# brdav/refign

Measured on AMD Instinct MI355X. Metric: image-pairs/s (align+seg fwd+bwd, 1080x1920), higher is better.
Workload: dtype bf16

## Files before the change

### refign_amd/csrc/kvpath.hip

```cpp
#include "common.h"
#include "elem.h"
#include "mfma.h"

namespace rfn {

constexpr int kKvBlocks = 3;
constexpr int kKvSmall = 128;
constexpr int kKvPack = 4096;
constexpr int kKvSPitch = 64 + 8;

template <int C, int R, int NB> struct KvGeom {
  static constexpr int ROWS = 32 * NB;
  static constexpr int KSTEP = C <= 128 ? 128 : 64;
  static constexpr int XP = KSTEP + 8, YP = C + 8;
  static constexpr int YBYTES = ROWS * YP * 2;
  static constexpr int XBYTES = R > 1 ? ROWS * XP * 2 : 0;
  static constexpr int WSCR = 32 * ((R > 1 && KSTEP > 64 ? KSTEP : 64) + 8) * 2;
  static constexpr int SBYTES = 4 * WSCR;
  static constexpr int LDS = YBYTES + 2 * XBYTES + SBYTES;
  static_assert(C % 64 == 0 && (R == 1 || (R * C) % KSTEP == 0), "a K-step never straddles a run of the gather");
  static_assert(LDS <= 160 * 1024, "LDS");
};

template <int DT, int C, int R, int NB>
__global__ __launch_bounds__(256) void kvpath_kernel(const uint16_t* __restrict__ X, const uint16_t* __restrict__ Wsr,
                                                     const uint16_t* __restrict__ bsr, const float* __restrict__ gamma,
                                                     const float* __restrict__ beta, float eps, const uint16_t* __restrict__ Wkv,
                                                     const uint16_t* __restrict__ bkv, unsigned char* __restrict__ kr,
                                                     unsigned char* __restrict__ vt, uint16_t* __restrict__ kvout, int B, int H,
                                                     int W, int Wr, int Nkv, int nkblk) {
  using E = Elem<DT>;
  using vec8 = typename E::vec8;
  using G = KvGeom<C, R, NB>;
  constexpr int kKvBlocks = NB, kKvRows = G::ROWS;
  constexpr int CB = C / 32, HEADS = C / 64, NCH = 2 * HEADS;
  constexpr int YP = G::YP;
  __shared__ __attribute__((aligned(16))) unsigned char smem[G::LDS];
  uint16_t* yt = (uint16_t*)smem;
  unsigned char* scr = smem + G::YBYTES + 2 * G::XBYTES;

  const int t = threadIdx.x, lane = t & 63, col = lane & 31, g = lane >> 5;
  const int wave = __builtin_amdgcn_readfirstlane(t >> 6);
  const int nblocks = B * nkblk, gb0 = blockIdx.x * kKvBlocks;
  auto row_of = [&](int tr, int& b, int& blk, int& row) {
    const int gb = gb0 + (tr >> 5);
    b = gb / nkblk;
    blk = gb - b * nkblk;
    row = blk * 32 + (tr & 31);
    return gb < nblocks && row < Nkv;
  };

  if constexpr (R > 1) {
    constexpr int KSTEP = G::KSTEP, XP = G::XP, NKS = KSTEP / 16, K1 = R * R * C;
    constexpr int PPR = KSTEP / 8, RPP = 256 / PPR, NI = kKvRows / RPP;
    constexpr int NCW = CB >= 4 ? (CB + 3) / 4 : 1, NTW = CB >= 4 ? kKvBlocks : (kKvBlocks + 1) / 2;
    static_assert(CB >= 4 || CB == 2, "wave map");
    const int sub = t % PPR, rb = t / PPR;
    unsigned xo[NI];
#pragma unroll
    for (int i = 0; i < NI; ++i) {
      int b, blk, row;
      const bool ok = row_of(rb + RPP * i, b, blk, row);
      const int oy = row / Wr, ox = row - oy * Wr;
      xo[i] = (ok ? (unsigned)(((b * H + oy * R) * W + ox * R) * C) : 0u) + sub * 8;
    }
    auto fetch_x = [&](int k0, u32x4(&rx)[NI]) {
      const int ry = k0 / (R * C);
      const unsigned off = (unsigned)(ry * W * C + (k0 - ry * R * C));
#pragma unroll
      for (int i = 0; i < NI; ++i) rx[i] = *(const u32x4*)(X + (xo[i] + off));
    };
    auto stash_x = [&](int buf, const u32x4(&rx)[NI]) {
      unsigned char* xs = smem + G::YBYTES + buf * G::XBYTES + (rb * XP + sub * 8) * 2;
#pragma unroll
      for (int i = 0; i < NI; ++i) *(u32x4*)(xs + RPP * i * XP * 2) = rx[i];
    };
    int cbc[NCW], tbc[NTW];
    bool cb_ok[NCW], tb_ok[NTW];
#pragma unroll
    for (int i = 0; i < NCW; ++i) {
      const int cb = CB >= 4 ? wave + 4 * i : (wave & 1);
      cb_ok[i] = cb < CB;
      cbc[i] = min(cb, CB - 1);
    }
#pragma unroll
    for (int j = 0; j < NTW; ++j) {
      const int tb = CB >= 4 ? j : (wave >> 1) + 2 * j;
      tb_ok[j] = tb < kKvBlocks;
      tbc[j] = min(tb, kKvBlocks - 1);
    }
    constexpr int WP = KSTEP + 8, PPW = KSTEP / 8, RPI = 64 / PPW;
    static_assert(32 / RPI == NKS, "instructions per block");
    const int wr = lane / PPW, wp = lane % PPW;
    const uint16_t* wrow[NCW];
#pragma unroll
    for (int i = 0; i < NCW; ++i) wrow[i] = Wsr + (long)(cbc[i] * 32 + wr) * K1 + wp * 8;
    auto fetch_w = [&](int k0, vec8(&wf)[NCW][NKS]) {
#pragma unroll
      for (int i = 0; i < NCW; ++i)
#pragma unroll
        for (int q = 0; q < NKS; ++q) wf[i][q] = *(const vec8*)(wrow[i] + (long)q * RPI * K1 + k0);
    };
    unsigned char* wscr = scr + wave * G::WSCR;
    auto to_frags = [&](const vec8(&raw)[NKS], vec8(&fr)[NKS]) {
      asm volatile("" ::: "memory");
#pragma unroll
      for (int q = 0; q < NKS; ++q) *(vec8*)(wscr + ((q * RPI + wr) * WP + wp * 8) * 2) = raw[q];
      asm volatile("" ::: "memory");
#pragma unroll
      for (int ks = 0; ks < NKS; ++ks) fr[ks] = *(const vec8*)(wscr + (col * WP + ks * 16 + 8 * g) * 2);
      asm volatile("" ::: "memory");
    };
    f32x16 acc[NCW][NTW];
#pragma unroll
    for (int i = 0; i < NCW; ++i)
#pragma unroll
      for (int j = 0; j < NTW; ++j)
#pragma unroll
        for (int r = 0; r < 16; ++r) acc[i][j][r] = 0.f;
    constexpr int nk = K1 / KSTEP;
    auto kstep = [&](int s, vec8(&cur)[NCW][NKS], vec8(&far)[NCW][NKS], const u32x4(&rnext)[NI], u32x4(&rfar)[NI]) {
      const bool more = s + 1 < nk;
      if (s + 2 < nk) {
        fetch_x((s + 2) * KSTEP, rfar);
        fetch_w((s + 2) * KSTEP, far);
      }
      const unsigned char* xs = smem + G::YBYTES + (s & 1) * G::XBYTES;
      auto xfrag = [&](int j, int ks) { return *(const vec8*)(xs + ((tbc[j] * 32 + col) * XP + ks * 16 + 8 * g) * 2); };
      vec8 xall[NCW > 1 ? NKS : 1][NTW];
      if constexpr (NCW > 1) {
#pragma unroll
        for (int ks = 0; ks < NKS; ++ks)
#pragma unroll
          for (int j = 0; j < NTW; ++j) xall[ks][j] = xfrag(j, ks);
      }
#pragma unroll
      for (int i = 0; i < NCW; ++i) {
        vec8 wfr[NKS];
        to_frags(cur[i], wfr);
#pragma unroll
        for (int ks = 0; ks < NKS; ++ks)
#pragma unroll
          for (int j = 0; j < NTW; ++j) acc[i][j] = E::mma(wfr[ks], NCW > 1 ? xall[NCW > 1 ? ks : 0][j] : xfrag(j, ks), acc[i][j]);
      }
      if (more) stash_x((s + 1) & 1, rnext);
      __syncthreads();
    };
    vec8 wf0[NCW][NKS], wf1[NCW][NKS], wf2[NCW][NKS];
    u32x4 rxa[NI], rxb[NI];
    static_assert(nk >= 2, "two steps in flight");
    fetch_x(0, rxa);
    fetch_w(0, wf0);
    fetch_x(KSTEP, rxb);
    fetch_w(KSTEP, wf1);
    stash_x(0, rxa);
    __syncthreads();
#pragma unroll 1
    for (int s = 0; s < nk; s += 6) {
      kstep(s, wf0, wf2, rxb, rxa);
      if (s + 1 < nk) kstep(s + 1, wf1, wf0, rxa, rxb);
      if (s + 2 < nk) kstep(s + 2, wf2, wf1, rxb, rxa);
      if (s + 3 < nk) kstep(s + 3, wf0, wf2, rxa, rxb);
      if (s + 4 < nk) kstep(s + 4, wf1, wf0, rxb, rxa);
      if (s + 5 < nk) kstep(s + 5, wf2, wf1, rxa, rxb);
    }
#pragma unroll
    for (int i = 0; i < NCW; ++i)
#pragma unroll
      for (int j = 0; j < NTW; ++j) {
        if (!(cb_ok[i] && tb_ok[j])) continue;
        const int tok = tbc[j] * 32 + col;
#pragma unroll
        for (int q = 0; q < 4; ++q) {
          const int n0 = cbc[i] * 32 + 8 * q + 4 * g;
          float bf[4];
          unpack4<DT>(*(const u32x2*)(bsr + n0), bf);
          *(u32x2*)(yt + tok * YP + n0) = pack4<DT>(acc[i][j][4 * q] + bf[0], acc[i][j][4 * q + 1] + bf[1],
                                                   acc[i][j][4 * q + 2] + bf[2], acc[i][j][4 * q + 3] + bf[3]);
        }
      }
    __syncthreads();
    {
      constexpr int LPR = C <= 64 ? 8 : (C <= 128 ? 16 : (C <= 256 ? 32 : 64)), RPW = 64 / LPR;
      const int ls = lane % LPR, grp = lane / LPR, c = ls * 8;
      const bool act = c < C;
      float gm[8], bt[8];
#pragma unroll
      for (int h = 0; h < 2; ++h) {
        const f32x4 a = *(const f32x4*)(gamma + (act ? c : 0) + 4 * h), b = *(const f32x4*)(beta + (act ? c : 0) + 4 * h);
#pragma unroll
        for (int e = 0; e < 4; ++e) {
          gm[4 * h + e] = a[e];
          bt[4 * h + e] = b[e];
        }
      }
      const float invC = 1.0f / (float)C;
#pragma unroll 1
      for (int it = 0; it < kKvRows / (4 * RPW); ++it) {
        uint16_t* p = yt + ((it * 4 + wave) * RPW + grp) * YP + (act ? c : 0);
        float v[8];
        if (act) load8<DT>(p, v);
        else {
#pragma unroll
          for (int i = 0; i < 8; ++i) v[i] = 0.0f;
        }
        float s = 0.0f;
#pragma unroll
        for (int i = 0; i < 8; ++i) s += v[i];
#pragma unroll
        for (int o = LPR / 2; o > 0; o >>= 1) s += __shfl_xor(s, o, 64);
        const float mu = s * invC;
        float q = 0.0f;
#pragma unroll
        for (int i = 0; i < 8; ++i) {
          const float d = act ? v[i] - mu : 0.0f;
          q = fmaf(d, d, q);
        }
#pragma unroll
        for (int o = LPR / 2; o > 0; o >>= 1) q += __shfl_xor(q, o, 64);
        const float rs = rsqrtf(q * invC + eps);
        if (act) {
          float o[8];
#pragma unroll
          for (int i = 0; i < 8; ++i) o[i] = fmaf((v[i] - mu) * rs, gm[i], bt[i]);
          const u32x2 lo = pack4<DT>(o[0], o[1], o[2], o[3]), hi = pack4<DT>(o[4], o[5], o[6], o[7]);
          *(u32x4*)p = u32x4{lo[0], lo[1], hi[0], hi[1]};
        }
      }
    }
    __syncthreads();
  } else {
    constexpr int PPR = C / 8;
    for (int p = t; p < kKvRows * PPR; p += 256) {
      const int tr = p / PPR, sub = p - tr * PPR;
      int b, blk, row;
      u32x4 v = {0u, 0u, 0u, 0u};
      if (row_of(tr, b, blk, row)) v = *(const u32x4*)(X + ((long)b * Nkv + row) * C + sub * 8);
      *(u32x4*)(yt + tr * YP + sub * 8) = v;
    }
    __syncthreads();
  }

  constexpr int NPASS = (NCH + 3) / 4;
#pragma unroll 1
  for (int pass = 0; pass < NPASS; ++pass) {
    const int hc = pass * 4 + wave;
    const bool hc_ok = hc < NCH;
    const int hcc = min(hc, NCH - 1);
    unsigned char* ws = scr + wave * G::WSCR;
    const int wr = lane >> 3, wp = lane & 7;
    const uint16_t* w2row = Wkv + (long)(hcc * 64 + wr) * C + wp * 8;
    auto fetch_w2 = [&](int k0, vec8(&wf)[2][4]) {
#pragma unroll
      for (int a = 0; a < 2; ++a)
#pragma unroll
        for (int q = 0; q < 4; ++q) wf[a][q] = *(const vec8*)(w2row + (long)(a * 32 + q * 8) * C + k0);
    };
    auto to_frags2 = [&](const vec8(&raw)[4], vec8(&fr)[4]) {
      asm volatile("" ::: "memory");
#pragma unroll
      for (int q = 0; q < 4; ++q) *(vec8*)(ws + ((q * 8 + wr) * kKvSPitch + wp * 8) * 2) = raw[q];
      asm volatile("" ::: "memory");
#pragma unroll
      for (int ks = 0; ks < 4; ++ks) fr[ks] = *(const vec8*)(ws + (col * kKvSPitch + ks * 16 + 8 * g) * 2);
      asm volatile("" ::: "memory");
    };
    f32x16 acc2[2][kKvBlocks];
#pragma unroll
    for (int a = 0; a < 2; ++a)
#pragma unroll
      for (int j = 0; j < kKvBlocks; ++j)
#pragma unroll
        for (int r = 0; r < 16; ++r) acc2[a][j][r] = 0.f;
    auto kstep2 = [&](int s, vec8(&cur)[2][4], vec8(&far)[2][4]) {
      if (s + 2 < HEADS) fetch_w2((s + 2) * 64, far);
      vec8 yf[4][kKvBlocks];
#pragma unroll
      for (int ks = 0; ks < 4; ++ks)
#pragma unroll
        for (int j = 0; j < kKvBlocks; ++j) yf[ks][j] = *(const vec8*)(yt + (j * 32 + col) * YP + s * 64 + ks * 16 + 8 * g);
#pragma unroll
      for (int a = 0; a < 2; ++a) {
        vec8 wfr[4];
        to_frags2(cur[a], wfr);
#pragma unroll
        for (int ks = 0; ks < 4; ++ks)
#pragma unroll
          for (int j = 0; j < kKvBlocks; ++j) acc2[a][j] = E::mma(wfr[ks], yf[ks][j], acc2[a][j]);
      }
    };
    vec8 v0[2][4], v1[2][4], v2[2][4];
    fetch_w2(0, v0);
    if (HEADS > 1) fetch_w2(64, v1);
#pragma unroll 1
    for (int s = 0; s < HEADS; s += 3) {
      kstep2(s, v0, v2);
      if (s + 1 < HEADS) kstep2(s + 1, v1, v0);
      if (s + 2 < HEADS) kstep2(s + 2, v2, v1);
    }
    const bool is_k = hc < HEADS;
#pragma unroll
    for (int j = 0; j < kKvBlocks; ++j) {
      int b, blk, row;
      const bool valid = row_of(j * 32 + col, b, blk, row);
      const bool live = hc_ok && gb0 + j < nblocks;
      const long pblk = ((long)(b * NCH + hcc) * nkblk + blk) * kKvPack;
#pragma unroll
      for (int a = 0; a < 2; ++a)
#pragma unroll
        for (int pr = 0; pr < 2; ++pr) {
          float ba[4], bb[4];
          const uint16_t* bp = bkv + hcc * 64 + a * 32 + 16 * pr + 4 * g;
          unpack4<DT>(*(const u32x2*)bp, ba);
          unpack4<DT>(*(const u32x2*)(bp + 8), bb);
          const u32x2 pa = pack4<DT>(acc2[a][j][8 * pr] + ba[0], acc2[a][j][8 * pr + 1] + ba[1], acc2[a][j][8 * pr + 2] + ba[2],
                                     acc2[a][j][8 * pr + 3] + ba[3]);
          const u32x2 pb = pack4<DT>(acc2[a][j][8 * pr + 4] + bb[0], acc2[a][j][8 * pr + 5] + bb[1], acc2[a][j][8 * pr + 6] + bb[2],
                                     acc2[a][j][8 * pr + 7] + bb[3]);
          auto r0 = __builtin_amdgcn_permlane32_swap(pa[0], pb[0], false, false);
          auto r1 = __builtin_amdgcn_permlane32_swap(pa[1], pb[1], false, false);
          const u32x4 o = valid ? u32x4{r0[0], r1[0], r0[1], r1[1]} : u32x4{0u, 0u, 0u, 0u};
          const int dc = a * 4 + 2 * pr + g;
          if (live && is_k) *(u32x4*)(kr + pblk + (dc * 32 + col) * 16) = o;
          if (live && valid && kvout != nullptr) *(u32x4*)(kvout + ((long)b * Nkv + row) * (2 * C) + hcc * 64 + dc * 8) = o;
          *(u32x4*)(ws + (col * kKvSPitch + dc * 8) * 2) = o;
        }
      __syncthreads();
      if (live && !is_k) {
        const uint16_t* sc = (const uint16_t*)ws + lane;
#pragma unroll
        for (int rq = 0; rq < 8; ++rq) {
          const unsigned h0 = sc[(4 * rq) * kKvSPitch], h1 = sc[(4 * rq + 1) * kKvSPitch], h2 = sc[(4 * rq + 2) * kKvSPitch],
                         h3 = sc[(4 * rq + 3) * kKvSPitch];
          *(u32x2*)(vt + pblk + (rq * 64 + lane) * 8) = u32x2{h0 | (h1 << 16), h2 | (h3 << 16)};
        }
      }
      __syncthreads();
    }
  }
}

template <int DT, int C, int R, int NB>
static int kvpath_launch(const void* x, const void* w_sr, const void* b_sr, const float* gamma, const float* beta, float eps,
                         const void* w_kv, const void* b_kv, void* k_rpack, void* v_tpack, void* kv_out, int B, int H, int W, int Nkv,
                         int nkblk, hipStream_t st) {
  const int tiles = cdiv((long)B * nkblk, NB);
  hipLaunchKernelGGL((kvpath_kernel<DT, C, R, NB>), dim3(tiles), dim3(256), 0, st, (const uint16_t*)x, (const uint16_t*)w_sr,
                     (const uint16_t*)b_sr, gamma, beta, eps, (const uint16_t*)w_kv, (const uint16_t*)b_kv, (unsigned char*)k_rpack,
                     (unsigned char*)v_tpack, (uint16_t*)kv_out, B, H, W, R > 1 ? W / R : 1, Nkv, nkblk);
  return check_launch("kvpath_kernel");
}

}

extern "C" int rfn_kv_path(const void* x, const void* w_sr, const void* b_sr, const float* gamma, const float* beta, float eps,
                           const void* w_kv, const void* b_kv, void* k_rpack, void* v_tpack, void* kv_out, int B, int H, int W, int C,
                           int r, int nkblk, int blocks_per_wg, int dtype, rfn_stream_t stream) {
  using namespace rfn;
  RFN_REQUIRE(x && w_kv && b_kv && k_rpack && v_tpack, "rfn_kv_path: null pointer");
  RFN_REQUIRE(r == 1 || (w_sr && b_sr && gamma && beta), "rfn_kv_path: r = %d needs the spatial-reduction and LayerNorm parameters", r);
  RFN_REQUIRE(B > 0 && H >= r && W >= r && r >= 1, "rfn_kv_path: B=%d H=%d W=%d r=%d", B, H, W, r);
  RFN_REQUIRE((long)B * H * W * C < (1L << 31), "rfn_kv_path: B*H*W*C = %ld (32-bit element offsets)", (long)B * H * W * C);
  const int Nkv = (H / r) * (W / r);
  RFN_REQUIRE(nkblk % 2 == 0 && (long)nkblk * 32 >= Nkv && (long)B * nkblk < (1L << 24),
              "rfn_kv_path: nkblk=%d (even, >= ceil(%d / 32))", nkblk, Nkv);
  hipStream_t st = (hipStream_t)stream;
  RFN_REQUIRE(blocks_per_wg == 0 || blocks_per_wg == 1 || blocks_per_wg == kKvBlocks, "rfn_kv_path: blocks_per_wg=%d (0, 1 or %d)",
              blocks_per_wg, kKvBlocks);
  const bool small = blocks_per_wg ? blocks_per_wg == 1 : cdiv((long)B * nkblk, kKvBlocks) < kKvSmall;
  return dt16(dtype, "rfn_kv_path", [&](auto dtc) {
    constexpr int DT = decltype(dtc)::value;
#define RFN_KV(CC, RR)                                                                                                   \
  if (C == CC && r == RR)                                                                                                \
    return small ? kvpath_launch<DT, CC, RR, 1>(x, w_sr, b_sr, gamma, beta, eps, w_kv, b_kv, k_rpack, v_tpack, kv_out, B, H, W, Nkv, \
                                                nkblk, st)                                                               \
                 : kvpath_launch<DT, CC, RR, kKvBlocks>(x, w_sr, b_sr, gamma, beta, eps, w_kv, b_kv, k_rpack, v_tpack, kv_out, B, H, \
                                                        W, Nkv, nkblk, st)
    RFN_KV(64, 8);
    RFN_KV(128, 4);
    RFN_KV(320, 2);
    RFN_KV(512, 1);
#undef RFN_KV
    return fail(RFN_EINVAL, "rfn_kv_path: (C, r) = (%d, %d): built for (64, 8), (128, 4), (320, 2), (512, 1)", C, r);
  });
}
```

Measured before the change: 17.73.

## Use eight waves per workgroup in the KV path for wide channel stages

For C >= 320 the KV-path kernel now launches 8 waves instead of 4. The spatial-reduction GEMM, LayerNorm and KV projection work is spread across the extra waves, and the weight prefetch is shortened to one step ahead to save registers. LayerNorm is unrolled over four rows so more work is in flight, per-wave pack barriers become compiler fences, and bias loads are hoisted. An optional s_memtime trace hook is added but compiled out by default. The extra waves trade register and LDS pressure and a shallower prefetch for more parallelism inside each block.

```diff
diff --git a/refign_amd/csrc/kvpath.hip b/refign_amd/csrc/kvpath.hip
--- a/refign_amd/csrc/kvpath.hip
+++ b/refign_amd/csrc/kvpath.hip
@@ -8,31 +8,38 @@
 constexpr int kKvSmall = 128;
 constexpr int kKvPack = 4096;
 constexpr int kKvSPitch = 64 + 8;
+constexpr int kKvStamps = 64;
 
 template <int C, int R, int NB> struct KvGeom {
+#ifdef RFN_KV_FOUR_WAVES
+  static constexpr int NW = 4;
+#else
+  static constexpr int NW = C >= 320 ? 8 : 4;
+#endif
   static constexpr int ROWS = 32 * NB;
   static constexpr int KSTEP = C <= 128 ? 128 : 64;
   static constexpr int XP = KSTEP + 8, YP = C + 8;
   static constexpr int YBYTES = ROWS * YP * 2;
   static constexpr int XBYTES = R > 1 ? ROWS * XP * 2 : 0;
   static constexpr int WSCR = 32 * ((R > 1 && KSTEP > 64 ? KSTEP : 64) + 8) * 2;
-  static constexpr int SBYTES = 4 * WSCR;
+  static constexpr int SBYTES = NW * WSCR;
   static constexpr int LDS = YBYTES + 2 * XBYTES + SBYTES;
   static_assert(C % 64 == 0 && (R == 1 || (R * C) % KSTEP == 0), "a K-step never straddles a run of the gather");
   static_assert(LDS <= 160 * 1024, "LDS");
 };
 
-template <int DT, int C, int R, int NB>
-__global__ __launch_bounds__(256) void kvpath_kernel(const uint16_t* __restrict__ X, const uint16_t* __restrict__ Wsr,
-                                                     const uint16_t* __restrict__ bsr, const float* __restrict__ gamma,
+template <int DT, int C, int R, int NB, bool TRACE = false>
+__global__ __launch_bounds__((64 * KvGeom<C, R, NB>::NW)) void kvpath_kernel(const uint16_t* __restrict__ X,
+                                                     const uint16_t* __restrict__ Wsr, const uint16_t* __restrict__ bsr, const float* __restrict__ gamma,
                                                      const float* __restrict__ beta, float eps, const uint16_t* __restrict__ Wkv,
                                                      const uint16_t* __restrict__ bkv, unsigned char* __restrict__ kr,
                                                      unsigned char* __restrict__ vt, uint16_t* __restrict__ kvout, int B, int H,
-                                                     int W, int Wr, int Nkv, int nkblk) {
+                                                     int W, int Wr, int Nkv, int nkblk, unsigned long long* __restrict__ trace) {
   using E = Elem<DT>;
   using vec8 = typename E::vec8;
   using G = KvGeom<C, R, NB>;
-  constexpr int kKvBlocks = NB, kKvRows = G::ROWS;
+  constexpr int kKvBlocks = NB, kKvRows = G::ROWS, NW = G::NW, NT = 64 * NW;
+  constexpr int AH = NW > 4 ? 1 : 2;
   constexpr int CB = C / 32, HEADS = C / 64, NCH = 2 * HEADS;
   constexpr int YP = G::YP;
   __shared__ __attribute__((aligned(16))) unsigned char smem[G::LDS];
@@ -50,17 +57,35 @@
     return gb < nblocks && row < Nkv;
   };
 
+  int tcount = 0;
+  auto stamp = [&]() {
+    if constexpr (TRACE) {
+      if (blockIdx.x == 0 && tcount < kKvStamps) {
+        unsigned long long tm;
+        __builtin_amdgcn_sched_barrier(0);
+        asm volatile("s_memtime %0\n\ts_waitcnt lgkmcnt(0)" : "=s"(tm)::"memory");
+        __builtin_amdgcn_sched_barrier(0);
+        if (lane == 0) trace[wave * kKvStamps + tcount] = tm;
+        ++tcount;
+      }
+    }
+  };
+  stamp();
+
   if constexpr (R > 1) {
     constexpr int KSTEP = G::KSTEP, XP = G::XP, NKS = KSTEP / 16, K1 = R * R * C;
-    constexpr int PPR = KSTEP / 8, RPP = 256 / PPR, NI = kKvRows / RPP;
-    constexpr int NCW = CB >= 4 ? (CB + 3) / 4 : 1, NTW = CB >= 4 ? kKvBlocks : (kKvBlocks + 1) / 2;
-    static_assert(CB >= 4 || CB == 2, "wave map");
+    constexpr int PPR = KSTEP / 8, RPP = NT / PPR, NI = (kKvRows + RPP - 1) / RPP;
+    constexpr bool XFULL = kKvRows % RPP == 0;
+    constexpr int NCW = CB >= 4 ? (CB + NW - 1) / NW : 1, NTW = CB >= 4 ? kKvBlocks : (kKvBlocks + 1) / 2;
+    static_assert((CB >= NW || CB == 2) && (NW == 4 || CB >= 4), "wave map");
     const int sub = t % PPR, rb = t / PPR;
     unsigned xo[NI];
+    bool xin[NI];
 #pragma unroll
     for (int i = 0; i < NI; ++i) {
       int b, blk, row;
-      const bool ok = row_of(rb + RPP * i, b, blk, row);
+      xin[i] = XFULL || rb + RPP * i < kKvRows;
+      const bool ok = row_of(rb + RPP * i, b, blk, row) && xin[i];
       const int oy = row / Wr, ox = row - oy * Wr;
       xo[i] = (ok ? (unsigned)(((b * H + oy * R) * W + ox * R) * C) : 0u) + sub * 8;
     }
@@ -73,13 +98,14 @@
     auto stash_x = [&](int buf, const u32x4(&rx)[NI]) {
       unsigned char* xs = smem + G::YBYTES + buf * G::XBYTES + (rb * XP + sub * 8) * 2;
 #pragma unroll
-      for (int i = 0; i < NI; ++i) *(u32x4*)(xs + RPP * i * XP * 2) = rx[i];
+      for (int i = 0; i < NI; ++i)
+        if (xin[i]) *(u32x4*)(xs + RPP * i * XP * 2) = rx[i];
     };
     int cbc[NCW], tbc[NTW];
     bool cb_ok[NCW], tb_ok[NTW];
 #pragma unroll
     for (int i = 0; i < NCW; ++i) {
-      const int cb = CB >= 4 ? wave + 4 * i : (wave & 1);
+      const int cb = CB >= 4 ? wave + NW * i : (wave & 1);
       cb_ok[i] = cb < CB;
       cbc[i] = min(cb, CB - 1);
     }
@@ -95,9 +121,9 @@
     const uint16_t* wrow[NCW];
 #pragma unroll
     for (int i = 0; i < NCW; ++i) wrow[i] = Wsr + (long)(cbc[i] * 32 + wr) * K1 + wp * 8;
-    auto fetch_w = [&](int k0, vec8(&wf)[NCW][NKS]) {
-#pragma unroll
-      for (int i = 0; i < NCW; ++i)
+    auto fetch_w = [&](auto nc, int k0, vec8(&wf)[NCW][NKS]) {
+#pragma unroll
+      for (int i = 0; i < decltype(nc)::value; ++i)
 #pragma unroll
         for (int q = 0; q < NKS; ++q) wf[i][q] = *(const vec8*)(wrow[i] + (long)q * RPI * K1 + k0);
     };
@@ -119,51 +145,72 @@
 #pragma unroll
         for (int r = 0; r < 16; ++r) acc[i][j][r] = 0.f;
     constexpr int nk = K1 / KSTEP;
-    auto kstep = [&](int s, vec8(&cur)[NCW][NKS], vec8(&far)[NCW][NKS], const u32x4(&rnext)[NI], u32x4(&rfar)[NI]) {
-      const bool more = s + 1 < nk;
-      if (s + 2 < nk) {
-        fetch_x((s + 2) * KSTEP, rfar);
-        fetch_w((s + 2) * KSTEP, far);
-      }
+    auto kstep = [&](auto nc, auto mode, int s, vec8(&cur)[NCW][NKS], vec8(&far)[NCW][NKS], const u32x4(&rnext)[NI],
+                     u32x4(&rfar)[NI]) {
+      constexpr int NC = decltype(nc)::value, MODE = decltype(mode)::value;
+      const bool more = MODE == 0 ? s + 1 < nk : MODE != 3;
+      if (MODE == 0 ? s + 2 < nk : MODE == 1) fetch_x((s + 2) * KSTEP, rfar);
+      if (MODE == 0 ? s + AH < nk : MODE != 3) fetch_w(nc, (s + AH) * KSTEP, far);
       const unsigned char* xs = smem + G::YBYTES + (s & 1) * G::XBYTES;
       auto xfrag = [&](int j, int ks) { return *(const vec8*)(xs + ((tbc[j] * 32 + col) * XP + ks * 16 + 8 * g) * 2); };
-      vec8 xall[NCW > 1 ? NKS : 1][NTW];
-      if constexpr (NCW > 1) {
+      constexpr bool XALL = NCW > 1 && NW == 4;
+      vec8 xall[XALL ? NKS : 1][NTW];
+      if constexpr (XALL) {
 #pragma unroll
         for (int ks = 0; ks < NKS; ++ks)
 #pragma unroll
           for (int j = 0; j < NTW; ++j) xall[ks][j] = xfrag(j, ks);
       }
 #pragma unroll
-      for (int i = 0; i < NCW; ++i) {
+      for (int i = 0; i < NC; ++i) {
         vec8 wfr[NKS];
         to_frags(cur[i], wfr);
 #pragma unroll
         for (int ks = 0; ks < NKS; ++ks)
 #pragma unroll
-          for (int j = 0; j < NTW; ++j) acc[i][j] = E::mma(wfr[ks], NCW > 1 ? xall[NCW > 1 ? ks : 0][j] : xfrag(j, ks), acc[i][j]);
+          for (int j = 0; j < NTW; ++j) acc[i][j] = E::mma(wfr[ks], XALL ? xall[XALL ? ks : 0][j] : xfrag(j, ks), acc[i][j]);
       }
       if (more) stash_x((s + 1) & 1, rnext);
       __syncthreads();
+      stamp();
     };
     vec8 wf0[NCW][NKS], wf1[NCW][NKS], wf2[NCW][NKS];
     u32x4 rxa[NI], rxb[NI];
     static_assert(nk >= 2, "two steps in flight");
-    fetch_x(0, rxa);
-    fetch_w(0, wf0);
-    fetch_x(KSTEP, rxb);
-    fetch_w(KSTEP, wf1);
-    stash_x(0, rxa);
-    __syncthreads();
+    auto product = [&](auto nc) {
+      fetch_x(0, rxa);
+      fetch_w(nc, 0, wf0);
+      fetch_x(KSTEP, rxb);
+      if constexpr (AH == 2) fetch_w(nc, KSTEP, wf1);
+      stash_x(0, rxa);
+      __syncthreads();
+      stamp();
+      using std::integral_constant;
+      if constexpr (AH == 1) {
+        static_assert(AH == 2 || nk % 2 == 0, "pairs of steps");
+        int s = 0;
 #pragma unroll 1
-    for (int s = 0; s < nk; s += 6) {
-      kstep(s, wf0, wf2, rxb, rxa);
-      if (s + 1 < nk) kstep(s + 1, wf1, wf0, rxa, rxb);
-      if (s + 2 < nk) kstep(s + 2, wf2, wf1, rxb, rxa);
-      if (s + 3 < nk) kstep(s + 3, wf0, wf2, rxa, rxb);
-      if (s + 4 < nk) kstep(s + 4, wf1, wf0, rxb, rxa);
-      if (s + 5 < nk) kstep(s + 5, wf2, wf1, rxa, rxb);
-    }
+        for (; s + 2 < nk; s += 2) {
+          kstep(nc, integral_constant<int, 1>{}, s, wf0, wf1, rxb, rxa);
+          kstep(nc, integral_constant<int, 1>{}, s + 1, wf1, wf0, rxa, rxb);
+        }
+        kstep(nc, integral_constant<int, 2>{}, s, wf0, wf1, rxb, rxa);
+        kstep(nc, integral_constant<int, 3>{}, s + 1, wf1, wf0, rxa, rxb);
+      } else {
+        constexpr integral_constant<int, 0> rt{};
+#pragma unroll 1
+        for (int s = 0; s < nk; s += 6) {
+          kstep(nc, rt, s, wf0, wf2, rxb, rxa);
+          if (s + 1 < nk) kstep(nc, rt, s + 1, wf1, wf0, rxa, rxb);
+          if (s + 2 < nk) kstep(nc, rt, s + 2, wf2, wf1, rxb, rxa);
+          if (s + 3 < nk) kstep(nc, rt, s + 3, wf0, wf2, rxa, rxb);
+          if (s + 4 < nk) kstep(nc, rt, s + 4, wf1, wf0, rxb, rxa);
+          if (s + 5 < nk) kstep(nc, rt, s + 5, wf2, wf1, rxa, rxb);
+        }
+      }
+    };
+    if (NW > 4 && NCW > 1 && !cb_ok[NCW - 1]) product(std::integral_constant<int, (NCW > 1 ? NCW - 1 : 1)>{});
+    else product(std::integral_constant<int, NCW>{});
 #pragma unroll
     for (int i = 0; i < NCW; ++i)
 #pragma unroll
@@ -180,6 +227,7 @@
         }
       }
     __syncthreads();
+    stamp();
     {
       constexpr int LPR = C <= 64 ? 8 : (C <= 128 ? 16 : (C <= 256 ? 32 : 64)), RPW = 64 / LPR;
       const int ls = lane % LPR, grp = lane / LPR, c = ls * 8;
@@ -195,43 +243,64 @@
         }
       }
       const float invC = 1.0f / (float)C;
+      constexpr int LNU = NW > 4 ? 4 : 1, ITER = kKvRows / (NW * RPW);
+      static_assert(ITER % LNU == 0, "rows in flight");
 #pragma unroll 1
-      for (int it = 0; it < kKvRows / (4 * RPW); ++it) {
-        uint16_t* p = yt + ((it * 4 + wave) * RPW + grp) * YP + (act ? c : 0);
-        float v[8];
-        if (act) load8<DT>(p, v);
-        else {
-#pragma unroll
-          for (int i = 0; i < 8; ++i) v[i] = 0.0f;
-        }
-        float s = 0.0f;
-#pragma unroll
-        for (int i = 0; i < 8; ++i) s += v[i];
-#pragma unroll
-        for (int o = LPR / 2; o > 0; o >>= 1) s += __shfl_xor(s, o, 64);
-        const float mu = s * invC;
-        float q = 0.0f;
-#pragma unroll
-        for (int i = 0; i < 8; ++i) {
-          const float d = act ? v[i] - mu : 0.0f;
-          q = fmaf(d, d, q);
-        }
-#pragma unroll
-        for (int o = LPR / 2; o > 0; o >>= 1) q += __shfl_xor(q, o, 64);
-        const float rs = rsqrtf(q * invC + eps);
+      for (int it = 0; it < ITER; it += LNU) {
+        uint16_t* p[LNU];
+        float v[LNU][8], s[LNU], q[LNU];
+#pragma unroll
+        for (int u = 0; u < LNU; ++u) {
+          p[u] = yt + (((it + u) * NW + wave) * RPW + grp) * YP + (act ? c : 0);
+          load8<DT>(p[u], v[u]);
+          s[u] = 0.0f;
+#pragma unroll
+          for (int i = 0; i < 8; ++i) {
+            v[u][i] = act ? v[u][i] : 0.0f;
+            s[u] += v[u][i];
+          }
+        }
+#pragma unroll
+        for (int o = LPR / 2; o > 0; o >>= 1)
+#pragma unroll
+          for (int u = 0; u < LNU; ++u) s[u] += __shfl_xor(s[u], o, 64);
+        float mu[LNU];
+#pragma unroll
+        for (int u = 0; u < LNU; ++u) {
+          mu[u] = s[u] * invC;
+          asm volatile("" : "+v"(mu[u]));
+          q[u] = 0.0f;
+#pragma unroll
+          for (int i = 0; i < 8; ++i) {
+            v[u][i] = act ? v[u][i] - mu[u] : 0.0f;
+            q[u] = fmaf(v[u][i], v[u][i], q[u]);
+          }
+        }
+#pragma unroll
+        for (int o = LPR / 2; o > 0; o >>= 1)
+#pragma unroll
+          for (int u = 0; u < LNU; ++u) q[u] += __shfl_xor(q[u], o, 64);
         if (act) {
-          float o[8];
-#pragma unroll
-          for (int i = 0; i < 8; ++i) o[i] = fmaf((v[i] - mu) * rs, gm[i], bt[i]);
-          const u32x2 lo = pack4<DT>(o[0], o[1], o[2], o[3]), hi = pack4<DT>(o[4], o[5], o[6], o[7]);
-          *(u32x4*)p = u32x4{lo[0], lo[1], hi[0], hi[1]};
+#pragma unroll
+          for (int u = 0; u < LNU; ++u) {
+            const float rs = rsqrtf(fmaf(q[u], invC, eps));
+            float o[8];
+#pragma unroll
+            for (int i = 0; i < 8; ++i) {
+              o[i] = fmaf(v[u][i] * rs, gm[i], bt[i]);
+              asm volatile("" : "+v"(o[i]));
+            }
+            const u32x2 lo = pack4<DT>(o[0], o[1], o[2], o[3]), hi = pack4<DT>(o[4], o[5], o[6], o[7]);
+            *(u32x4*)p[u] = u32x4{lo[0], lo[1], hi[0], hi[1]};
+          }
         }
       }
     }
     __syncthreads();
+    stamp();
   } else {
     constexpr int PPR = C / 8;
-    for (int p = t; p < kKvRows * PPR; p += 256) {
+    for (int p = t; p < kKvRows * PPR; p += NT) {
       const int tr = p / PPR, sub = p - tr * PPR;
       int b, blk, row;
       u32x4 v = {0u, 0u, 0u, 0u};
@@ -239,13 +308,19 @@
       *(u32x4*)(yt + tr * YP + sub * 8) = v;
     }
     __syncthreads();
+    stamp();
   }
 
-  constexpr int NPASS = (NCH + 3) / 4;
+  constexpr int NPASS = (NCH + NW - 1) / NW;
+  auto pack_sync = [&]() {
+    if constexpr (NW == 4) __syncthreads();
+    else asm volatile("" ::: "memory");
+  };
 #pragma unroll 1
   for (int pass = 0; pass < NPASS; ++pass) {
-    const int hc = pass * 4 + wave;
+    const int hc = pass * NW + wave;
     const bool hc_ok = hc < NCH;
+    if (NW > 4 && !hc_ok) break;
     const int hcc = min(hc, NCH - 1);
     unsigned char* ws = scr + wave * G::WSCR;
     const int wr = lane >> 3, wp = lane & 7;
@@ -272,13 +347,18 @@
       for (int j = 0; j < kKvBlocks; ++j)
 #pragma unroll
         for (int r = 0; r < 16; ++r) acc2[a][j][r] = 0.f;
-    auto kstep2 = [&](int s, vec8(&cur)[2][4], vec8(&far)[2][4]) {
-      if (s + 2 < HEADS) fetch_w2((s + 2) * 64, far);
-      vec8 yf[4][kKvBlocks];
-#pragma unroll
-      for (int ks = 0; ks < 4; ++ks)
-#pragma unroll
-        for (int j = 0; j < kKvBlocks; ++j) yf[ks][j] = *(const vec8*)(yt + (j * 32 + col) * YP + s * 64 + ks * 16 + 8 * g);
+    auto kstep2 = [&](auto mode, int s, vec8(&cur)[2][4], vec8(&far)[2][4]) {
+      constexpr int MODE = decltype(mode)::value;
+      if (MODE == 0 ? s + AH < HEADS : MODE == 1) fetch_w2((s + AH) * 64, far);
+      auto yfrag = [&](int j, int ks) { return *(const vec8*)(yt + (j * 32 + col) * YP + s * 64 + ks * 16 + 8 * g); };
+      constexpr bool YALL = NW == 4;
+      vec8 yf[YALL ? 4 : 1][kKvBlocks];
+      if constexpr (YALL) {
+#pragma unroll
+        for (int ks = 0; ks < 4; ++ks)
+#pragma unroll
+          for (int j = 0; j < kKvBlocks; ++j) yf[ks][j] = yfrag(j, ks);
+      }
 #pragma unroll
       for (int a = 0; a < 2; ++a) {
         vec8 wfr[4];
@@ -286,19 +366,49 @@
 #pragma unroll
         for (int ks = 0; ks < 4; ++ks)
 #pragma unroll
-          for (int j = 0; j < kKvBlocks; ++j) acc2[a][j] = E::mma(wfr[ks], yf[ks][j], acc2[a][j]);
+          for (int j = 0; j < kKvBlocks; ++j) acc2[a][j] = E::mma(wfr[ks], YALL ? yf[YALL ? ks : 0][j] : yfrag(j, ks), acc2[a][j]);
       }
     };
     vec8 v0[2][4], v1[2][4], v2[2][4];
     fetch_w2(0, v0);
-    if (HEADS > 1) fetch_w2(64, v1);
+    if (AH == 2 && HEADS > 1) fetch_w2(64, v1);
+    if constexpr (AH == 1) {
+      constexpr std::integral_constant<int, 1> req{};
+      constexpr std::integral_constant<int, 3> last{};
+      int s = 0;
 #pragma unroll 1
-    for (int s = 0; s < HEADS; s += 3) {
-      kstep2(s, v0, v2);
-      if (s + 1 < HEADS) kstep2(s + 1, v1, v0);
-      if (s + 2 < HEADS) kstep2(s + 2, v2, v1);
-    }
+      for (; s + 2 < HEADS; s += 2) {
+        kstep2(req, s, v0, v1);
+        kstep2(req, s + 1, v1, v0);
+      }
+      if constexpr (HEADS % 2 == 0) {
+        kstep2(req, s, v0, v1);
+        kstep2(last, s + 1, v1, v0);
+      } else {
+        kstep2(last, s, v0, v1);
+      }
+    } else {
+      constexpr std::integral_constant<int, 0> rt{};
+#pragma unroll 1
+      for (int s = 0; s < HEADS; s += 3) {
+        kstep2(rt, s, v0, v2);
+        if (s + 1 < HEADS) kstep2(rt, s + 1, v1, v0);
+        if (s + 2 < HEADS) kstep2(rt, s + 2, v2, v1);
+      }
+    }
+    stamp();
     const bool is_k = hc < HEADS;
+    u32x2 bpre[NW > 4 ? 2 : 1][2][2];
+    if constexpr (NW > 4) {
+#pragma unroll
+      for (int a = 0; a < 2; ++a)
+#pragma unroll
+        for (int pr = 0; pr < 2; ++pr) {
+          const uint16_t* bp = bkv + hcc * 64 + a * 32 + 16 * pr + 4 * g;
+          bpre[a][pr][0] = *(const u32x2*)bp;
+          bpre[a][pr][1] = *(const u32x2*)(bp + 8);
+        }
+    }
 #pragma unroll
     for (int j = 0; j < kKvBlocks; ++j) {
       int b, blk, row;
@@ -311,8 +421,8 @@
         for (int pr = 0; pr < 2; ++pr) {
           float ba[4], bb[4];
           const uint16_t* bp = bkv + hcc * 64 + a * 32 + 16 * pr + 4 * g;
-          unpack4<DT>(*(const u32x2*)bp, ba);
-          unpack4<DT>(*(const u32x2*)(bp + 8), bb);
+          unpack4<DT>(NW > 4 ? bpre[NW > 4 ? a : 0][pr][0] : *(const u32x2*)bp, ba);
+          unpack4<DT>(NW > 4 ? bpre[NW > 4 ? a : 0][pr][1] : *(const u32x2*)(bp + 8), bb);
           const u32x2 pa = pack4<DT>(acc2[a][j][8 * pr] + ba[0], acc2[a][j][8 * pr + 1] + ba[1], acc2[a][j][8 * pr + 2] + ba[2],
                                      acc2[a][j][8 * pr + 3] + ba[3]);
           const u32x2 pb = pack4<DT>(acc2[a][j][8 * pr + 4] + bb[0], acc2[a][j][8 * pr + 5] + bb[1], acc2[a][j][8 * pr + 6] + bb[2],
@@ -325,7 +435,7 @@
           if (live && valid && kvout != nullptr) *(u32x4*)(kvout + ((long)b * Nkv + row) * (2 * C) + hcc * 64 + dc * 8) = o;
           *(u32x4*)(ws + (col * kKvSPitch + dc * 8) * 2) = o;
         }
-      __syncthreads();
+      pack_sync();
       if (live && !is_k) {
         const uint16_t* sc = (const uint16_t*)ws + lane;
 #pragma unroll
@@ -335,24 +445,28 @@
           *(u32x2*)(vt + pblk + (rq * 64 + lane) * 8) = u32x2{h0 | (h1 << 16), h2 | (h3 << 16)};
         }
       }
-      __syncthreads();
-    }
+      pack_sync();
+    }
+    stamp();
   }
 }
 
+#ifndef RFN_KVPATH_KERNEL_ONLY
 template <int DT, int C, int R, int NB>
 static int kvpath_launch(const void* x, const void* w_sr, const void* b_sr, const float* gamma, const float* beta, float eps,
                          const void* w_kv, const void* b_kv, void* k_rpack, void* v_tpack, void* kv_out, int B, int H, int W, int Nkv,
                          int nkblk, hipStream_t st) {
   const int tiles = cdiv((long)B * nkblk, NB);
-  hipLaunchKernelGGL((kvpath_kernel<DT, C, R, NB>), dim3(tiles), dim3(256), 0, st, (const uint16_t*)x, (const uint16_t*)w_sr,
+  hipLaunchKernelGGL((kvpath_kernel<DT, C, R, NB>), dim3(tiles), dim3(64 * KvGeom<C, R, NB>::NW), 0, st, (const uint16_t*)x, (const uint16_t*)w_sr,
                      (const uint16_t*)b_sr, gamma, beta, eps, (const uint16_t*)w_kv, (const uint16_t*)b_kv, (unsigned char*)k_rpack,
-                     (unsigned char*)v_tpack, (uint16_t*)kv_out, B, H, W, R > 1 ? W / R : 1, Nkv, nkblk);
+                     (unsigned char*)v_tpack, (uint16_t*)kv_out, B, H, W, R > 1 ? W / R : 1, Nkv, nkblk, nullptr);
   return check_launch("kvpath_kernel");
 }
+#endif
 
 }
 
+#ifndef RFN_KVPATH_KERNEL_ONLY
 extern "C" int rfn_kv_path(const void* x, const void* w_sr, const void* b_sr, const float* gamma, const float* beta, float eps,
                            const void* w_kv, const void* b_kv, void* k_rpack, void* v_tpack, void* kv_out, int B, int H, int W, int C,
                            int r, int nkblk, int blocks_per_wg, int dtype, rfn_stream_t stream) {
@@ -384,3 +498,4 @@
     return fail(RFN_EINVAL, "rfn_kv_path: (C, r) = (%d, %d): built for (64, 8), (128, 4), (320, 2), (512, 1)", C, r);
   });
 }
+#endif
```

Result: no change. 17.86, median of 6 (+0.7%).
